# Parskatt/RoMa

Hardware: NVIDIA H100
Metric: image-pairs/sec match()+sample() 560->864 (higher is better)
Workload: dtype f32 (activations f32; GEMM operands as split-f16 pairs hi + 2^-11 lo on wgmma, f32 accumulate: fp32-class)

## Files before the change

include/romab200.h:

```cpp
#ifndef ROMAB200_H
#define ROMAB200_H

#include <stdint.h>

#ifdef __cplusplus
extern "C" {
#endif

#define ROMAB200_ABI_VERSION 4

enum rb_dtype { RB_F32 = 0, RB_F16 = 1, RB_BF16 = 2, RB_F16S = 3, RB_F64 = 4 };
enum rb_act { RB_ACT_NONE = 0, RB_ACT_RELU = 1, RB_ACT_GELU = 2 };
enum rb_rowmap { RB_ROWMAP_NONE = 0, RB_ROWMAP_PAD_KEEP = 1, RB_ROWMAP_PAD_TO_COMPACT = 2, RB_ROWMAP_SEGMENT = 3 };
enum rb_epi { RB_EPI_LINEAR = 0, RB_EPI_COSKERNEL = 1 };
enum rb_backend { RB_BACKEND_AUTO = 0, RB_BACKEND_SIMT = 1, RB_BACKEND_TCGEN05 = 2 };

int romab200_abi_version(void);
const char* romab200_last_error(void);
unsigned long long romab200_launch_count(void);
int romab200_device_ok(void);

typedef struct {
    const void* A; const void* B; void* C;
    int32_t M, N, K;
// ... 39 lines not shown

typedef struct {
    const void* src; void* dst; int64_t rows; int32_t cols; int64_t lds, ldd; int32_t dtype_src, dtype_dst;
    const float* row_scale; int32_t row_scale_reciprocal;
} rb_copy2d_args;
int romab200_copy2d(const rb_copy2d_args* args, void* stream);

typedef struct {
    const void* src; void* dst; const int32_t* src_index; const int32_t* dst_index;
    int32_t count; int64_t row_bytes, ld_src, ld_dst; int32_t src_rows, dst_rows;
} rb_gather_rows_args;
int romab200_gather_rows(const rb_gather_rows_args* args, void* stream);

typedef struct {
    const float* x; void* dst; int64_t rows; int32_t cols; int64_t ldx, ldd; const float* row_norm;
    int32_t layout_b;
} rb_split_args;
int romab200_split_f16x3(const rb_split_args* args, void* stream);

typedef struct {
    const float* x; void* hi; void* lo; int64_t rows; int32_t cols; int64_t ldx, ldd; const float* row_norm;
} rb_split_pair_args;
int romab200_split_f16s(const rb_split_pair_args* args, void* stream);

typedef struct {
    const float* image; void* out; const float* weight ; const float* bias ;
    int32_t batch, height, width, cout; int32_t dtype_out;
    void* out_lo;
} rb_conv_first_args;
int romab200_conv3x3_first(const rb_conv_first_args* args, void* stream);
typedef struct { const void* in; void* out; int32_t batch, height, width, channels, dtype;
                 const void* in_lo; void* out_lo;  } rb_maxpool_args;
int romab200_maxpool2x2_padded(const rb_maxpool_args* args, void* stream);

typedef struct { const float* image; void* out; int32_t batch, height, width, patch; int64_t ldo; int32_t dtype_out; } rb_im2col_args;
int romab200_im2col_patch(const rb_im2col_args* args, void* stream);
typedef struct { const float* patch; const float* cls; const float* pos; float* tokens; int32_t batch, npatch, dim; } rb_tokens_args;
int romab200_assemble_tokens(const rb_tokens_args* args, void* stream);

typedef struct {
    float* W; int32_t n, nrhs, batch; int64_t ldw, stride;
    void* workspace; int64_t workspace_bytes;
    int32_t algo;
} rb_gp_solve_args;
int romab200_gp_solve(const rb_gp_solve_args* args, void* stream);
typedef struct { const void* logits; float* state; int64_t rows; int64_t ldl; int32_t res; int32_t dtype; } rb_cls_args;
int romab200_cls_to_flow_refine(const rb_cls_args* args, void* stream);

typedef struct {
    const void* feat; int64_t ldf; int32_t n_img, y_shift;
    const float* state; void* d; int64_t ldd;
    int32_t D, h, w, cf, emb, radius; int32_t dtype;
    const float* emb_weight ; const float* emb_bias; float disp_scale;
    const float* grid_x; const float* grid_y;
    const float* win_x; const float* win_y;
    void* tile_done; int32_t tile_done_len;
    const float* corr_table; int64_t ld_corr_table;
} rb_refiner_prologue_args;
int romab200_refiner_prologue(const rb_refiner_prologue_args* args, void* stream);

typedef struct {
    const void* f0; const void* f1; int64_t ldf0, ldf1; int64_t f0_img_stride, f1_img_stride;
    const float* flow; int64_t ldflow; void* out; int64_t ldo;
    int32_t batch, h, w, c, radius; float scale; int32_t dtype_f, dtype_out;
    int32_t n_img, y_shift;
    const float* win_x; const float* win_y;
// ... 543 lines not shown
```

roma_b200/cabi.py:

```python
from __future__ import annotations

import ctypes
import os
import re
from typing import Dict

import torch

HERE = os.path.dirname(os.path.abspath(__file__))
HEADER = os.path.join(os.path.dirname(HERE), "include", "romab200.h")
LIB_PATH = os.path.join(HERE, "lib", "libromab200.so")

RB_F32, RB_F16, RB_BF16, RB_F16S, RB_F64 = 0, 1, 2, 3, 4
ACT_NONE, ACT_RELU, ACT_GELU = 0, 1, 2
ROWMAP_NONE, ROWMAP_PAD_KEEP, ROWMAP_PAD_TO_COMPACT, ROWMAP_SEGMENT = 0, 1, 2, 3
EPI_LINEAR, EPI_COSKERNEL = 0, 1
BACKEND_AUTO, BACKEND_SIMT, BACKEND_TCGEN05 = 0, 1, 2
SAMPLE_IDENTITY, SAMPLE_THRESHOLD, SAMPLE_BALANCE = 0, 1, 2

DTYPE_CODE = {torch.float32: RB_F32, torch.float16: RB_F16, torch.bfloat16: RB_BF16}

_CTYPES = {
    "int32_t": ctypes.c_int32, "int64_t": ctypes.c_int64, "uint64_t": ctypes.c_uint64, "float": ctypes.c_float, "double": ctypes.c_double,
}
# ... 66 lines not shown
                           "(there is no CPU or PyTorch fallback for the CUDA path)")
    lib = ctypes.CDLL(path)
    lib.romab200_last_error.restype = ctypes.c_char_p
    lib.romab200_abi_version.restype = ctypes.c_int
    lib.romab200_device_ok.restype = ctypes.c_int
    lib.romab200_launch_count.restype = ctypes.c_ulonglong
    for fn in FUNCTIONS:
        getattr(lib, fn)
    _lib = lib
    return lib


def _stream():
    return ctypes.c_void_p(torch.cuda.current_stream().cuda_stream)


launch_count = 0

_CODE_DTYPE = {RB_F32: torch.float32, RB_F16: torch.float16, RB_BF16: torch.bfloat16, RB_F16S: torch.float16, RB_F64: torch.float64}
_F32 = torch.float32
_F64 = torch.float64
_FIELD_DTYPES = {
    "rb_gemm_args": {"A": "dtype_ab", "B": "dtype_ab", "A_lo": torch.float16, "B_lo": torch.float16, "C": "dtype_c", "C_lo": torch.float16,
                     "R": "dtype_r", "bias": _F32, "col_scale": _F32, "norm_a": _F32, "norm_b": _F32},
    "rb_layernorm_args": {"x": "dtype_x", "y": "dtype_y", "y_lo": torch.float16, "gamma": _F32, "beta": _F32},
    "rb_softmax_args": {"s": "dtype", "out_hi": torch.float16, "out_lo": torch.float16},
    "rb_flash_attn_args": {"qkv": "dtype", "out": "dtype", "qkv_lo": torch.float16, "out_lo": torch.float16},
    "rb_rownorm_args": {"x": "dtype", "out": _F32},
    "rb_copy2d_args": {"src": "dtype_src", "dst": "dtype_dst", "row_scale": _F32},
    "rb_gather_rows_args": {"src_index": torch.int32, "dst_index": torch.int32},
    "rb_split_pair_args": {"x": _F32, "hi": torch.float16, "lo": torch.float16, "row_norm": _F32},
    "rb_conv_first_args": {"image": _F32, "out": "dtype_out", "out_lo": torch.float16, "weight": _F32, "bias": _F32},
    "rb_maxpool_args": {"in": "dtype", "out": "dtype", "in_lo": torch.float16, "out_lo": torch.float16},
    "rb_im2col_args": {"image": _F32, "out": "dtype_out"},
    "rb_tokens_args": {"patch": _F32, "cls": _F32, "pos": _F32, "tokens": _F32},
    "rb_gp_solve_args": {"W": _F32},
    "rb_cls_args": {"logits": "dtype", "state": _F32},
    "rb_refiner_prologue_args": {"feat": "dtype", "state": _F32, "d": "dtype", "emb_weight": _F32, "emb_bias": _F32, "grid_x": _F32, "grid_y": _F32,
                                 "win_x": _F32, "win_y": _F32, "tile_done": torch.uint8, "corr_table": _F32},
    "rb_local_corr_args": {"f0": "dtype_f", "f1": "dtype_f", "flow": _F32, "out": "dtype_out", "win_x": _F32, "win_y": _F32},
    "rb_local_corr_warp_args": {"f0": _F32, "f1": _F32, "warp": _F32, "out": _F32},
    "rb_dwconv_args": {"in": "dtype", "weight": _F32, "bias": _F32, "out_lo": torch.float16},
    "rb_refiner_block_small_args": {"in": "dtype", "out": "dtype", "dw_weight": _F32, "dw_bias": _F32, "pw_weight_host": _F32, "pw_bias_host": _F32},
    "rb_refiner_block_c144_args": {"in": "dtype", "out": "dtype", "dw_weight": _F32, "dw_bias": _F32, "pw_weight": "dtype", "pw_bias": _F32},
    "rb_refiner_block_c144_split_args": {"in": _F32, "out": _F32, "dw_weight": _F32, "dw_bias": _F32, "pw_weight": torch.float16,
                                         "pw_weight_lo": torch.float16, "pw_bias": _F32},
    "rb_refiner_tail_args": {"d": "dtype", "weight": _F32, "bias": _F32, "state": _F32, "delta_out": _F32},
    "rb_resize_args": {"in": _F32, "out": _F32},
    "rb_match_epilogue_args": {"state": _F32, "coarse_state": _F32, "warp": _F32, "cert": _F32, "grid_x": _F32, "grid_y": _F32},
    "rb_kde_args": {"x": _F32, "density": _F32, "workspace": _F32},
    "rb_preprocess_args": {"in": torch.uint8, "tmp": torch.uint8, "out_u8": torch.uint8, "out": _F32, "bounds_x": torch.int32, "kk_x": torch.int32,
                           "bounds_y": torch.int32, "kk_y": torch.int32},
    "rb_sample_args": {"values": _F32, "out_idx": torch.int32, "out_weights": _F32, "keys": _F32, "scratch": torch.int32, "seed_dev": torch.int64},
    "rb_sample_gather_args": {"matches": _F32, "certainty": _F32, "idx": torch.int32, "out_matches": _F32, "out_certainty": _F32},
    "rb_tiny_conv_args": {"in": _F32, "out": _F32, "weight": _F32, "bias": _F32, "col_scale": _F32, "R": _F32},
    "rb_tiny_gray_args": {"in": _F32, "out": _F32},
    "rb_tiny_avgpool_args": {"in": _F32, "out": _F32},
    "rb_tiny_add3_args": {"a": _F32, "b": _F32, "c": _F32, "out": _F32},
    "rb_tiny_pos_embed_args": {"f0": _F32, "f1": _F32, "state": _F32, "grid_x": _F32, "grid_y": _F32, "grid_lr_x": _F32, "grid_lr_y": _F32},
    "rb_tiny_warp_concat_args": {"f0": _F32, "f1": _F32, "state": _F32, "out": _F32},
    "rb_tiny_epilogue_args": {"state": _F32, "warp": _F32, "cert": _F32, "grid_x": _F32, "grid_y": _F32},
    "rb_keypoints_sample_args": {"x": _F32, "warp": _F32, "cert": _F32, "x_to_B": _F32, "cert_out": _F32},
    "rb_keypoints_mnn_args": {"x_A_to_B": _F32, "cert_A": _F32, "x_B": _F32, "workspace": _F32, "offsets": torch.int64, "inds_A": torch.int64,
                              "inds_B": torch.int64},
    "rb_jpeg_args": {"stream": torch.uint8, "desc": torch.int64, "tables": torch.int32, "comp": torch.uint8, "chunks": torch.int32,
                     "istart": torch.int32, "exits": torch.int64, "counts": torch.int32, "coef": torch.int16, "state": torch.int32,
# ... 45 lines not shown
                        "x2": _F64, "prob": _F32},
    "rb_dense_geometric_dist_args": {"depth0": "depth_dtype", "depth1": "depth_dtype", "T": _F64, "K0": _F64, "K1": _F64, "dense_matches": _F32,
                                     "gd": _F64, "prob": _F32, "partial_sum": _F64, "partial_cnt": torch.int32, "pair_sum": _F64,
                                     "pair_cnt": torch.int64, "pck": _F32, "epe": _F64},
    "rb_dense_tri_args": {"pairs": torch.int64, "warp": _F32, "certainty": _F32, "image_sizes": torch.int32, "cameras": _F64,
                          "registered": torch.uint8, "images": torch.int32, "depth": _F32, "score": _F32, "source": torch.int64,
                          "elem_depth": _F32, "partial": torch.int32, "pair_counts": torch.int64},
    "rb_dense_fuse_args": {"image_sizes": torch.int32, "cameras": _F64, "registered": torch.uint8, "nbr_offsets": torch.int64,
                           "nbrs": torch.int32, "depth": _F32, "score": _F32, "colors": torch.uint8, "color_offsets": torch.int64,
                           "color_sizes": torch.int32, "tile_scan": torch.int64, "points": _F64, "rgb": torch.uint8, "image": torch.int32,
                           "pixel": torch.int64, "num_views": torch.int32, "point_score": _F32},
}
_STRIDED_FIELDS = {"rb_keypoints_sample_args": {"warp", "cert"}, "rb_dense_geometric_dist_args": {"dense_matches"}}
_HOST_FIELDS = {"rb_refiner_block_small_args": {"pw_weight_host", "pw_bias_host"}}


def _gemm_min_elems(kw):
    b0, b1 = kw.get("batch0", 1) or 1, kw.get("batch1", 1) or 1
    M, N, K, nt = kw["M"], kw["N"], kw["K"], kw.get("ntaps", 1) or 1
    offa = (b0 - 1) * kw.get("sa0", 0) + (b1 - 1) * kw.get("sa1", 0)
    offb = (b0 - 1) * kw.get("sb0", 0) + (b1 - 1) * kw.get("sb1", 0)
    offc = (b0 - 1) * kw.get("sc0", 0) + (b1 - 1) * kw.get("sc1", 0)
    a = offa + ((kw.get("a_rows") or M) - 1) * kw["lda"] + K // nt
    b = offb + ((K - 1) * kw["ldb"] + N if kw.get("trans_b", 0) else (N - 1) * kw["ldb"] + K)
    rows_out = M
    if kw.get("rowmap", 0) == ROWMAP_PAD_TO_COMPACT:
        rows_out = M // (kw["pad_h"] * kw["pad_w"]) * (kw["pad_h"] - 2) * (kw["pad_w"] - 2)
    elif kw.get("rowmap", 0) == ROWMAP_SEGMENT:
        rows_out = (M - 1) // kw["seg_in"] * kw["seg_out"] + (M - 1) % kw["seg_in"] + kw.get("seg_off", 0) + 1
    c = offc + (rows_out - 1) * kw["ldc"] + N
    return {"A": a, "A_lo": a, "B": b, "B_lo": b, "C": c, "C_lo": c}


def _copy2d_min_elems(kw):
    return {"src": (kw["rows"] - 1) * kw["lds"] + kw["cols"], "dst": (kw["rows"] - 1) * kw["ldd"] + kw["cols"]}


def _gather_rows_min_elems(kw):
    out = {}
    for k, rows, ld in (("src", "src_rows", "ld_src"), ("dst", "dst_rows", "ld_dst")):
        if isinstance(kw.get(k), torch.Tensor):
            out[k] = -(-((kw[rows] - 1) * kw[ld] + kw["row_bytes"]) // kw[k].element_size())
    return out


def _sample_min_elems(kw):
    b, n, k, rep = max(kw.get("batch", 1), 1), kw["n"], kw["k"], max(kw.get("repeats", 0), 1)
    return {"values": ((b - 1) // rep) * (kw.get("stride") or n) + n, "keys": b * n, "scratch": b * 2056, "out_idx": b * k, "out_weights": b * k,
            "seed_dev": (b - 1) * kw.get("seed_stride", 0) + 1}


def _sample_gather_min_elems(kw):
    items, k, rows = kw["items"], kw["k"], ((kw["items"] - 1) // max(kw.get("repeats", 0), 1) + 1) * kw["n"]
    return {"matches": 4 * rows, "certainty": rows, "idx": items * k, "out_matches": 4 * items * k, "out_certainty": items * k}


def _match_graph_keypoints_min_elems(kw):
    sides, img = kw["num_pairs"] * kw["n"], kw["num_images"] + 1
    return {"pairs": 2 * kw["num_pairs"], "matches": 4 * sides, "certainty": sides, "image_sizes": 2 * kw["num_images"], "cell_start": img,
            "tile_start": img, "grid_bits": kw["grid_cells"], "grid_g": kw["grid_cells"], "tile_scan": kw["grid_tiles"] + 1, "kp_offsets": img,
            "keypoints": 2 * kw["kp_capacity"], "kp_scores": kw["kp_capacity"], "sid": 2 * sides}


def _match_graph_pairs_min_elems(kw):
    sides, cap = kw["num_pairs"] * kw["n"], kw.get("match_capacity", 0)
    return {"sid": 2 * sides, "certainty": sides, "scratch": kw.get("scratch_bytes", 0), "match_offsets": kw["num_pairs"] + 1,
# ... 64 lines not shown
        total = kw["x"].numel() // 2
        out.update(images=kw["num_list"], out_offsets=kw["num_list"] + 1, X=3 * total)
    return out


def _undistort_min_elems(kw):
    return {"kp_offsets": kw["num_images"] + 1, "keypoints": 2 * kw["num_rows"], "intrinsics": 4 * kw["num_images"], "out": 2 * kw["num_rows"],
            "clamped": 1}


def _twoview_min_elems(kw):
    B, total = kw["batch"], kw["mask"].numel()
    return {"offsets": B + 1, "x0": 2 * total, "x1": 2 * total, "xn": 4 * total, "K": 18 * B, "R": 9 * B, "t": 3 * B, "ok": B,
            "angle": total, "num_good": B, "median_angle": B, "forward": B}


def _dense_tri_min_elems(kw):
    P, N, C, n = kw["num_pairs"], kw["num_images"], kw["chunk"], kw["H"] * kw["W"]
    return {"pairs": 2 * P, "warp": 8 * C * n, "certainty": 2 * C * n, "image_sizes": 2 * N, "cameras": N * RB_DENSE_CAM, "registered": N,
            "images": kw["num_list"], "depth": N * n, "score": N * n, "source": N * n, "elem_depth": 2 * C * n,
            "partial": 2 * C * RB_DENSE_MAX_CTAS * RB_DENSE_REASONS, "pair_counts": P * RB_DENSE_REASONS}


def _dense_fuse_min_elems(kw):
    N, n, M = kw["num_images"], kw["H"] * kw["W"], kw.get("num_points", 0)
    out = {"image_sizes": 2 * N, "cameras": N * RB_DENSE_CAM, "registered": N, "nbr_offsets": N + 1, "depth": N * n, "score": N * n,
           "color_offsets": N + 1, "color_sizes": 2 * N, "tile_scan": N * (-(-n // RB_DENSE_TILE)) + 1, "points": 3 * M, "rgb": 3 * M,
           "image": M, "pixel": M, "num_views": M, "point_score": M}
    if kw.get("colors") is not None:
        out["colors"] = kw["color_bytes"]
    return out


_MIN_ELEMS = {"rb_gemm_args": _gemm_min_elems, "rb_copy2d_args": _copy2d_min_elems, "rb_gather_rows_args": _gather_rows_min_elems,
              "rb_sample_args": _sample_min_elems, "rb_sample_gather_args": _sample_gather_min_elems,
              "rb_match_graph_keypoints_args": _match_graph_keypoints_min_elems, "rb_match_graph_pairs_args": _match_graph_pairs_min_elems,
              "rb_tracks_args": _tracks_min_elems, "rb_verify_args": _verify_min_elems, "rb_tri_args": _tri_min_elems,
              "rb_ba_args": _ba_min_elems, "rb_ba_groups_args": _ba_groups_min_elems, "rb_abspose_args": _abspose_min_elems,
              "rb_register_args": _register_min_elems,
              "rb_twoview_args": _twoview_min_elems, "rb_undistort_args": _undistort_min_elems,
              "rb_dense_tri_args": _dense_tri_min_elems, "rb_dense_fuse_args": _dense_fuse_min_elems}


def _validate(fn_name, struct_name, kw):
    table = _FIELD_DTYPES.get(struct_name, {})
    cur = torch.cuda.current_device() if torch.cuda.is_available() else None
    mins = _MIN_ELEMS[struct_name](kw) if struct_name in _MIN_ELEMS else {}
    strided = _STRIDED_FIELDS.get(struct_name, ())
    host = _HOST_FIELDS.get(struct_name, ())
    for k, v in kw.items():
        if not isinstance(v, torch.Tensor):
            if v is not None and k in _PTR_FIELDS[struct_name]:
                raise TypeError(f"{fn_name}: pointer field `{k}` takes a tensor or None, not {type(v).__name__} "
                                "(pass an operand that starts inside a buffer as a view, packing.at)")
            continue
        if k in host:
            if v.device.type != "cpu":
                raise RuntimeError(f"{fn_name}: argument `{k}` is read on the host, it must be a CPU tensor (got one on {v.device})")
        elif not v.is_cuda or (cur is not None and v.device.index != cur):
            raise RuntimeError(f"{fn_name}: argument `{k}` lives on {v.device}, expected the current CUDA device cuda:{cur}")
        if k not in strided and not v.is_contiguous():
            raise RuntimeError(f"{fn_name}: argument `{k}` is not contiguous (shape {tuple(v.shape)}, strides {v.stride()})")
        want = table.get(k)
        if isinstance(want, str):
            want = _CODE_DTYPE.get(kw.get(want))
        if want is not None and v.dtype != want:
            raise RuntimeError(f"{fn_name}: argument `{k}` has dtype {v.dtype}, the call describes it as {want}")
# ... 40 lines not shown
```

roma_b200/csrc/gemm_tc.cu:

```cuda
#include "tma.cuh"
#include "wgmma.cuh"

namespace rb {

struct TcParams {
    int M, N, K;
    int batch1;
    int ntaps, k_per_tap; int tap_rows[9];
    int tiles_m, tiles_n, total_tiles;
    int band_m;
    int n_zero_to;
    int64_t sc0, sc1, sr0, sr1, sna0, snb0;
    Epilogue epi;
};

constexpr int TC_BM = 128, TC_BK = 64;
constexpr int TC_THREADS = 384;
constexpr int TC_CW = 32, TC_SP = 40;
constexpr int TC_STAGING = 2 * 64 * TC_SP * 4;

template <int BN, bool SPLIT> struct TcCfg {
    static constexpr int NOPS = SPLIT ? 2 : 1;
    static constexpr int A_BYTES = TC_BM * TC_BK * 2;
    static constexpr int B_BYTES = BN * TC_BK * 2;
// ... 85 lines not shown
            v[k] = expf((v[k] * s - 1.0f) * e.inv_t);
            if (m == n + k) v[k] += e.diag_add;
        }
    } else {
#pragma unroll
        for (int k = 0; k < 8; ++k) v[k] = __fmul_rn(e.alpha, v[k]);
        if (e.bias) {
#pragma unroll
            for (int k = 0; k < 8; ++k) v[k] = __fadd_rn(v[k], cb[k]);
        }
        if (e.act == RB_ACT_RELU) {
#pragma unroll
            for (int k = 0; k < 8; ++k) v[k] = fmaxf(v[k], 0.0f);
        } else if (e.act == RB_ACT_GELU) {
#pragma unroll
            for (int k = 0; k < 8; ++k) v[k] = gelu_erf(v[k]);
        }
        if (e.col_scale) {
#pragma unroll
            for (int k = 0; k < 8; ++k) v[k] = __fmul_rn(v[k], cs[k]);
        }
        if (e.R) {
            float r[8];
            load8(e.R, orow * e.ldr + n, e.dtype_r, nv, r);
#pragma unroll
            for (int k = 0; k < 8; ++k) v[k] = __fadd_rn(v[k], r[k]);
        }
    }
    if (nv < 8) {
#pragma unroll
        for (int k = 0; k < 8; ++k) if (k >= nv) v[k] = 0.f;
    }
    store8(e, orow * e.ldc + n, cnt, v);
}

__device__ __forceinline__ void tile_coords(const TcParams& p, int w, int& z, int& mt, int& nt) {
    const int per_z = p.tiles_m * p.tiles_n;
    z = w / per_z;
    const int r = w - z * per_z;
    const int m_lo = r / (p.band_m * p.tiles_n) * p.band_m;
    const int rows = min(p.band_m, p.tiles_m - m_lo);
    const int rb = r - m_lo * p.tiles_n;
    nt = rb / rows;
    mt = m_lo + (rb - nt * rows);
}

template <int BN, bool SPLIT, bool BF16, int TB>
__global__ void __launch_bounds__(TC_THREADS, 1)
gemm_tc_kernel(const __grid_constant__ CUtensorMap map_a, const __grid_constant__ CUtensorMap map_b,
               const __grid_constant__ CUtensorMap map_a_lo, const __grid_constant__ CUtensorMap map_b_lo, const TcParams p) {
    using Cfg = TcCfg<BN, SPLIT>;
    constexpr int STAGES = Cfg::STAGES;
    constexpr int A_BYTES = Cfg::A_BYTES, B_BYTES = Cfg::B_BYTES;
    constexpr int OFF_A_LO = A_BYTES, OFF_B = Cfg::NOPS * A_BYTES, OFF_B_LO = Cfg::NOPS * A_BYTES + B_BYTES;
    extern __shared__ uint8_t smem_raw[];
    uint8_t* smem = smem_raw + ((1024u - ((uint32_t)__cvta_generic_to_shared(smem_raw) & 1023u)) & 1023u);
    float* staging = reinterpret_cast<float*>(smem + STAGES * Cfg::STAGE_BYTES);
    uint64_t* full_bar = reinterpret_cast<uint64_t*>(smem + STAGES * Cfg::STAGE_BYTES + TC_STAGING);
    uint64_t* empty_bar = full_bar + STAGES;

    const int warp = threadIdx.x >> 5, lane = threadIdx.x & 31;
    const int kblocks = (p.K + TC_BK - 1) / TC_BK;

    if (threadIdx.x == 0) {
        for (int s = 0; s < STAGES; ++s) { mbar_init(&full_bar[s], 1); mbar_init(&empty_bar[s], 2); }
        asm volatile("fence.mbarrier_init.release.cluster;" ::: "memory");
// ... 53 lines not shown
            wgmma_fence();
#pragma unroll
            for (int k = 0; k < TC_BK / 16; ++k) {
                const uint32_t koff_a = wg * (64 * 128) + k * 32;
                const uint32_t koff_b = TB ? k * 2048 : k * 32;
                const uint32_t lbo_b = TB ? 64 * 128 : 16;
                const uint64_t a_hi = gmma_desc(st + koff_a, 16, 1024);
                const uint64_t b_hi = gmma_desc(st + OFF_B + koff_b, lbo_b, 1024);
                const int accum = (kb | k) != 0;
                Wgmma<BN, BF16>::template ss<TB>(acc, a_hi, b_hi, accum);
                if constexpr (SPLIT) {
                    const uint64_t a_lo = gmma_desc(st + OFF_A_LO + koff_a, 16, 1024);
                    const uint64_t b_lo = gmma_desc(st + OFF_B_LO + koff_b, lbo_b, 1024);
                    Wgmma<BN, BF16>::template ss<TB>(acc2, a_hi, b_lo, accum);
                    Wgmma<BN, BF16>::template ss<TB>(acc2, a_lo, b_hi, 1);
                }
            }
            wgmma_commit();
            wgmma_wait<1>();
            if (prev >= 0 && t == 0) mbar_arrive(&empty_bar[prev]);
            prev = s;
        }
        wgmma_wait<0>();
        wgmma_fence_regs(acc);
        if constexpr (SPLIT) wgmma_fence_regs(acc2);
        if (t == 0) mbar_arrive(&empty_bar[prev]);

        Epilogue e = p.epi;
        e.C = (char*)e.C + (z0 * p.sc0 + z1 * p.sc1) * dtype_size(e.dtype_c);
        if (e.C_lo) e.C_lo = (char*)e.C_lo + (z0 * p.sc0 + z1 * p.sc1) * 2;
        if (e.R) e.R = (const char*)e.R + (z0 * p.sr0 + z1 * p.sr1) * dtype_size(e.dtype_r);
        if (e.norm_a) e.norm_a += z0 * p.sna0;
        if (e.norm_b) e.norm_b += z0 * p.snb0;
        float* stg = staging + wg * (64 * TC_SP);
        const int fr = (t >> 5) * 16 + ((t & 31) >> 2), fc = 2 * (t & 3);
        const int g = t & 3, rr = t >> 2;
        int mrow[2]; int64_t orow[2]; float na[2] = {0.f, 0.f};
#pragma unroll
        for (int h = 0; h < 2; ++h) {
            mrow[h] = m0 + wg * 64 + rr + 32 * h;
            orow[h] = mrow[h] < e.M ? e.map_row(mrow[h]) : -1;
            if (orow[h] >= 0 && e.epi == RB_EPI_COSKERNEL) na[h] = e.norm_a[mrow[h]];
        }
        constexpr int NCH = (BN + TC_CW - 1) / TC_CW;
#pragma unroll 1
        for (int ch = 0; ch < NCH; ++ch) {
            if (n0 + ch * TC_CW >= p.n_zero_to) break;
            bar_named(1 + wg, 128);
#pragma unroll
            for (int c = 0; c < NCH; ++c) {
                if (c != ch) continue;
#pragma unroll
                for (int jj = 0; jj < TC_CW / 8; ++jj) {
                    const int j = c * (TC_CW / 8) + jj;
                    if (j >= BN / 8) break;
#pragma unroll
                    for (int h = 0; h < 2; ++h) {
                        float v0 = acc[4 * j + 2 * h], v1 = acc[4 * j + 2 * h + 1];
                        if constexpr (SPLIT) {
                            v0 = fmaf(acc2[4 * j + 2 * h], 1.0f / RB_SPLIT_SCALE, v0);
                            v1 = fmaf(acc2[4 * j + 2 * h + 1], 1.0f / RB_SPLIT_SCALE, v1);
                        }
                        *reinterpret_cast<float2*>(stg + (fr + 8 * h) * TC_SP + 8 * jj + fc) = make_float2(v0, v1);
                    }
                }
            }
            bar_named(1 + wg, 128);
            const int n = n0 + ch * TC_CW + 8 * g;
            if (ch * TC_CW + 8 * g >= BN || n >= p.n_zero_to) continue;
            const int cnt = min(8, p.n_zero_to - n);
            float cb[8], cs[8];
            const float* colb = e.epi == RB_EPI_COSKERNEL ? e.norm_b : e.bias;
#pragma unroll
            for (int k = 0; k < 8; ++k) {
                const bool in = n + k < e.N;
                cb[k] = colb && in ? colb[n + k] : 0.f;
                cs[k] = e.col_scale && in ? e.col_scale[n + k] : 0.f;
            }
#pragma unroll
            for (int h = 0; h < 2; ++h) {
                if (orow[h] < 0) continue;
                const float* src = stg + (rr + 32 * h) * TC_SP + 8 * g;
                const int q = (rr & 1) * 4;
                const float4 a = *reinterpret_cast<const float4*>(src + q), b = *reinterpret_cast<const float4*>(src + (4 - q));
                float v[8];
                if (q == 0) { v[0] = a.x; v[1] = a.y; v[2] = a.z; v[3] = a.w; v[4] = b.x; v[5] = b.y; v[6] = b.z; v[7] = b.w; }
                else        { v[0] = b.x; v[1] = b.y; v[2] = b.z; v[3] = b.w; v[4] = a.x; v[5] = a.y; v[6] = a.z; v[7] = a.w; }
                epilogue8(e, mrow[h], n, orow[h], cnt, cb, cs, na[h], v);
            }
        }
    }
}

static int make_map(CUtensorMap* map, const void* base, int dtype, uint64_t inner, uint64_t rows, uint64_t pitch_elems, uint64_t b1,
                    uint64_t s1_elems, uint64_t b0, uint64_t s0_elems, uint32_t box_inner, uint32_t box_rows) {
    RB_REQUIRE(((uintptr_t)base) % 16 == 0 && (pitch_elems * 2) % 16 == 0, "gemm_tc: operand base/pitch must be 16-byte aligned (pitch %llu elems)", (unsigned long long)pitch_elems);
    RB_REQUIRE((b1 <= 1 || (s1_elems * 2) % 16 == 0) && (b0 <= 1 || (s0_elems * 2) % 16 == 0), "gemm_tc: batch strides must be 16-byte aligned");
    cuuint64_t dims[4] = {inner, rows, b1 > 0 ? b1 : 1, b0 > 0 ? b0 : 1};
    cuuint64_t strides[3] = {pitch_elems * 2, (b1 > 1 ? s1_elems : pitch_elems * rows) * 2, (b0 > 1 ? s0_elems : pitch_elems * rows) * 2};
    cuuint32_t box[4] = {box_inner, box_rows, 1, 1};
    return encode_tiled(map, "gemm_tc", tma_dtype(dtype), 4, base, dims, strides, box,
                        CU_TENSOR_MAP_SWIZZLE_128B);
}

struct TcMaps { CUtensorMap a, b, a_lo, b_lo; };

template <int BN, bool SPLIT, bool BF16, int TB>
static int launch_tc(const TcMaps& maps, TcParams& p, int zdim, int max_ctas, cudaStream_t st) {
    using Cfg = TcCfg<BN, SPLIT>;
    auto kernel = gemm_tc_kernel<BN, SPLIT, BF16, TB>;
    if (ensure_smem<gemm_tc_kernel<BN, SPLIT, BF16, TB>>(Cfg::SMEM, "gemm_tc")) return 1;
    p.tiles_m = (p.M + TC_BM - 1) / TC_BM;
    p.tiles_n = (p.N + BN - 1) / BN;
    const long long total = (long long)p.tiles_m * p.tiles_n * zdim;
    RB_REQUIRE(total < (1ll << 31), "gemm_tc: too many tiles");
    p.total_tiles = (int)total;
    int resident = sm_count();
    if (max_ctas > 0 && max_ctas < resident) resident = max_ctas;
    const int grid = p.total_tiles < resident ? p.total_tiles : resident;
    const int64_t a_bytes = (int64_t)p.M * (p.ntaps > 1 ? p.k_per_tap : p.K) * Cfg::NOPS * 2;
    const int64_t b_bytes = (int64_t)p.N * p.K * Cfg::NOPS * 2;
    const bool bands = p.tiles_n > 1 && 2 * a_bytes > l2_bytes() && 2 * b_bytes <= l2_bytes();
// ... 52 lines not shown
        else if (a->N <= 144) BN = 144;
        else if (a->N <= 192) BN = 192;
        else {
            const int w192 = (a->N + 191) / 192 * 192 - a->N, w256 = (a->N + 255) / 256 * 256 - a->N;
            BN = (w192 + a->N / 20 < w256) ? 192 : 256;
        }
        if (((int64_t)((a->M + 127) / 128) * ((a->N + BN - 1) / BN) * zdim) < sm_count() * 2 / 3) BN = 128;
    }
    TcMaps maps;
    const uint64_t a_inner = p.ntaps > 1 ? p.k_per_tap : a->K;
    if (make_map(&maps.a, a->A, a->dtype_ab, a_inner, a_rows, a->lda, p.batch1, a->sa1, batch0, a->sa0, TC_BK, TC_BM)) return 1;
    if (split && make_map(&maps.a_lo, a->A_lo, a->dtype_ab, a_inner, a_rows, a->lda, p.batch1, a->sa1, batch0, a->sa0, TC_BK, TC_BM)) return 1;
    if (!a->trans_b) {
        if (make_map(&maps.b, a->B, a->dtype_ab, a->K, a->N, a->ldb, p.batch1, a->sb1, batch0, a->sb0, TC_BK, BN)) return 1;
        if (split && make_map(&maps.b_lo, a->B_lo, a->dtype_ab, a->K, a->N, a->ldb, p.batch1, a->sb1, batch0, a->sb0, TC_BK, BN)) return 1;
    } else {
        if (make_map(&maps.b, a->B, a->dtype_ab, a->N, a->K, a->ldb, p.batch1, a->sb1, batch0, a->sb0, 64, TC_BK)) return 1;
        if (split && make_map(&maps.b_lo, a->B_lo, a->dtype_ab, a->N, a->K, a->ldb, p.batch1, a->sb1, batch0, a->sb0, 64, TC_BK)) return 1;
    }
    if (!split) { maps.a_lo = maps.a; maps.b_lo = maps.b; }
    {
        const int es_c = dtype_size(a->dtype_c);
        const bool align_ok = ((uintptr_t)a->C) % 16 == 0 && (a->ldc * es_c) % 16 == 0 && (p.batch1 <= 1 || (a->sc1 * es_c) % 16 == 0) &&
                              (batch0 <= 1 || (a->sc0 * es_c) % 16 == 0) && (a->dtype_c != RB_F16S || ((uintptr_t)a->C_lo) % 16 == 0);
        const bool rowmap_ok = a->rowmap == RB_ROWMAP_NONE || a->rowmap == RB_ROWMAP_PAD_KEEP;
        const int gran = 16 / es_c;
        p.n_zero_to = align_ok && rowmap_ok && !a->R ? (a->N + gran - 1) / gran * gran : a->N;
    }
    if (split) return dispatch_tc<true, false>(BN, a->trans_b, maps, p, zdim, a->max_ctas, stream);
    return bf16 ? dispatch_tc<false, true>(BN, a->trans_b, maps, p, zdim, a->max_ctas, stream)
                : dispatch_tc<false, false>(BN, a->trans_b, maps, p, zdim, a->max_ctas, stream);
}

}
```

roma_b200/engine.py:

```python
from __future__ import annotations

import math
import os
from contextlib import contextmanager
from typing import Optional

import torch
import torch.nn.functional as F

from . import arch, cabi, sampling
from .cabi import call
from .cache import BufferArena
from .packing import PackedWeights, Split, at, pad8

PRECISIONS = {"fp32": torch.float32, "fp32_simt": torch.float32, "fp16": torch.float16, "bf16": torch.bfloat16}
F16S = cabi.RB_F16S


class Engine(BufferArena):
    def __init__(self, matcher_sd, dino_sd, device, precision: str = "fp32"):
        if precision not in PRECISIONS:
            raise ValueError(f"precision must be one of {list(PRECISIONS)}")
        super().__init__(device)
        if self.device.type != "cuda":
# ... 80 lines not shown
        if self._lane == "side" and self.side_ctas:
            args["max_ctas"] = self.side_ctas
        args.update(kw)
        if (self.split and dtype_ab is None) or isinstance(A, Split):
            if not isinstance(A, Split):
                assert args["batch0"] * args["batch1"] == 1 and lda % 8 == 0, "batched fp32 operands are split by the caller"
                A = self.split_pair(A, args.get("a_rows") or M, K // args["ntaps"], lda)
            if not isinstance(B, Split):
                assert args["batch0"] * args["batch1"] == 1 and ldb % 8 == 0
                tb = args.get("trans_b", 0)
                B = self.split_pair(B, K if tb else N, N if tb else K, ldb, name=f"splitb.{self._lane}.{(K if tb else N) * ldb}")
            dtype_ab = F16S
            args.update(A=A.hi, A_lo=A.lo, B=B.hi, B_lo=B.lo)
            if isinstance(C, Split):
                args.update(C=C.hi, C_lo=C.lo)
                dtype_c = F16S
            else:
                args.update(C=C)
        else:
            args.update(A=A, B=B, C=C)
        args["dtype_ab"] = self.dt if dtype_ab is None else dtype_ab
        args["dtype_c"] = self.dt if dtype_c is None else dtype_c
        if self.gemm_profile is None:
            call("romab200_gemm", "rb_gemm_args", **args)
            return
        start, end = torch.cuda.Event(enable_timing=True), torch.cuda.Event(enable_timing=True)
        start.record()
        call("romab200_gemm", "rb_gemm_args", **args)
        end.record()
        flops = 2.0 * M * N * K * args["batch0"] * args["batch1"]
        backend = {cabi.RB_F32: "simt", F16S: "tcgen05-split"}.get(args["dtype_ab"], "tcgen05")
        self.gemm_profile.append((backend, flops, start, end, (M, N, K, args["batch0"] * args["batch1"]), args.get("epi", cabi.EPI_LINEAR)))

    def layernorm(self, x, y, gb, rows, cols, eps, dtype_y=None):
        if isinstance(y, Split):
            call("romab200_layernorm", "rb_layernorm_args", x=x, y=y.hi, y_lo=y.lo, gamma=gb[0], beta=gb[1], rows=rows, cols=cols,
                 ldx=cols, ldy=cols, dtype_x=cabi.RB_F32, dtype_y=F16S, eps=eps)
            return
        call("romab200_layernorm", "rb_layernorm_args", x=x, y=y, gamma=gb[0], beta=gb[1], rows=rows, cols=cols,
             ldx=cols, ldy=cols, dtype_x=cabi.RB_F32, dtype_y=self.dt if dtype_y is None else dtype_y, eps=eps)

    def copy2d(self, src, dst, rows, cols, lds, ldd, ds, dd):
        call("romab200_copy2d", "rb_copy2d_args", src=src, dst=dst, rows=rows, cols=cols, lds=lds, ldd=ldd,
             dtype_src=ds, dtype_dst=dd)

    def vgg(self, image: torch.Tensor, tag: str):
        E, _, H, W = image.shape
        taps = {}
        layers = self.w.vgg
        h, w = H, W
        mk = (lambda name, shape: self.sbuf(name, shape, zero=True)) if self.split else (lambda name, shape: self.buf(name, shape, zero=True))
        cur = mk(f"vgg{tag}.s1.in", (E, h + 2, w + 2, 64))
        if self.split:
            call("romab200_conv3x3_first", "rb_conv_first_args", image=image, out=cur.hi, out_lo=cur.lo, weight=layers[0]["w"], bias=layers[0]["b"],
                 batch=E, height=h, width=w, cout=64, dtype_out=F16S)
        else:
            call("romab200_conv3x3_first", "rb_conv_first_args", image=image, out=cur, weight=layers[0]["w"], bias=layers[0]["b"],
                 batch=E, height=h, width=w, cout=64, dtype_out=self.dt)
        li, scale = 1, 1
        for nconv in (1, 2, 4, 4):
            for j in range(nconv):
                L = layers[li]
                li += 1
                nxt = mk(f"vgg{tag}.s{scale}.p{j % 2}", (E, h + 2, w + 2, L["cout"]))
                rows = E * (h + 2) * (w + 2)
                taps_rows = [(ky - 1) * (w + 2) + (kx - 1) for ky in range(3) for kx in range(3)]
                self.gemm(cur, L["w"], nxt, rows, L["cout"], 9 * L["cin"], L["cin"], 9 * L["cin"], L["cout"],
                          ntaps=9, tap_rows=taps_rows, a_rows=rows, bias=L["b"], act=cabi.ACT_RELU,
                          rowmap=cabi.ROWMAP_PAD_KEEP, pad_h=h + 2, pad_w=w + 2)
                cur = nxt
            taps[scale] = (cur, h, w)
            if self.debug is not None:
                self.debug[f"{tag}.vgg{scale}"] = (cur.join() if self.split else cur.float())[:, 1:h + 1, 1:w + 1].clone()
            if scale == 8:
                break
            c = layers[li - 1]["cout"]
            pooled = mk(f"vgg{tag}.s{scale * 2}.in", (E, h // 2 + 2, w // 2 + 2, c))
            if self.split:
                call("romab200_maxpool2x2_padded", "rb_maxpool_args", **{"in": cur.hi}, in_lo=cur.lo, out=pooled.hi, out_lo=pooled.lo,
                     batch=E, height=h, width=w, channels=c, dtype=F16S)
            else:
                call("romab200_maxpool2x2_padded", "rb_maxpool_args", **{"in": cur}, out=pooled, batch=E, height=h, width=w,
                     channels=c, dtype=self.dt)
            cur, h, w, scale = pooled, h // 2, w // 2, scale * 2
        return taps

    def attention(self, qkv, out, Bn, N, heads, dim, tag):
        d = dim // heads
        if self.dtype != torch.float32 and self.use_flash_attn:
            with self.stage(f"  attn.{tag}"):
                call("romab200_flash_attn", "rb_flash_attn_args", qkv=qkv, out=out, ld_qkv=3 * dim, ld_out=dim, batch=Bn, n_tokens=N,
                     heads=heads, head_dim=d, dtype=self.dt)
            return
        npad = pad8(N)
        ld = 3 * dim
        if self.split and d == 64 and self.use_flash_attn:
            with self.stage(f"  attn.{tag}"):
                call("romab200_flash_attn", "rb_flash_attn_args", qkv=qkv.hi, qkv_lo=qkv.lo, out=out.hi, out_lo=out.lo, ld_qkv=ld, ld_out=dim,
                     batch=Bn, n_tokens=N, heads=heads, head_dim=d, dtype=F16S)
            return
        if self.split:
            S = self.buf(f"attn.scores.{tag}", (Bn, heads, N, npad), dtype=torch.float32)
# ... 433 lines not shown
```

Baseline: 17.63.

## Add halo-tiled implicit-GEMM conv3x3 kernel for split-f16 VGG layers

Adds a dedicated wgmma conv3x3 kernel for VGG layers with cin 64 or 128. Each CTA loads one spatial 8x16 halo tile (hi and lo planes) into shared memory once via 4D TMA and reuses it across all nine taps and all output-channel tiles. Weights stream through an mbarrier ring driven by a producer warp. The goal is to cut redundant global re-reads of the A operand that the generic tap-row GEMM does per tap. The shared epilogue is factored into a helper. Risks are shared-memory pressure limiting stage depth, and wasted work on partial tiles at image edges.

New measurement: 17.75 (median of 6 runs). Within noise of the previous version (+0.7%).

```diff
diff --git a/include/romab200.h b/include/romab200.h
--- a/include/romab200.h
+++ b/include/romab200.h
@@ -95,6 +95,16 @@
 typedef struct { const void* in; void* out; int32_t batch, height, width, channels, dtype;
                  const void* in_lo; void* out_lo;  } rb_maxpool_args;
 int romab200_maxpool2x2_padded(const rb_maxpool_args* args, void* stream);
+typedef struct {
+    const void* in; const void* in_lo;
+    const void* weight; const void* weight_lo;
+    const float* bias;
+    void* out; void* out_lo;
+    int32_t batch, height, width, cin, cout;
+    int32_t act;
+    int32_t max_ctas;
+} rb_conv3x3_split_args;
+int romab200_conv3x3_split(const rb_conv3x3_split_args* args, void* stream);
 
 typedef struct { const float* image; void* out; int32_t batch, height, width, patch; int64_t ldo; int32_t dtype_out; } rb_im2col_args;
 int romab200_im2col_patch(const rb_im2col_args* args, void* stream);
diff --git a/roma_b200/cabi.py b/roma_b200/cabi.py
--- a/roma_b200/cabi.py
+++ b/roma_b200/cabi.py
@@ -122,6 +122,8 @@
     "rb_split_pair_args": {"x": _F32, "hi": torch.float16, "lo": torch.float16, "row_norm": _F32},
     "rb_conv_first_args": {"image": _F32, "out": "dtype_out", "out_lo": torch.float16, "weight": _F32, "bias": _F32},
     "rb_maxpool_args": {"in": "dtype", "out": "dtype", "in_lo": torch.float16, "out_lo": torch.float16},
+    "rb_conv3x3_split_args": {"in": torch.float16, "in_lo": torch.float16, "weight": torch.float16, "weight_lo": torch.float16, "bias": _F32,
+                              "out": torch.float16, "out_lo": torch.float16},
     "rb_im2col_args": {"image": _F32, "out": "dtype_out"},
     "rb_tokens_args": {"patch": _F32, "cls": _F32, "pos": _F32, "tokens": _F32},
     "rb_gp_solve_args": {"W": _F32},
@@ -233,6 +235,12 @@
     return {"A": a, "A_lo": a, "B": b, "B_lo": b, "C": c, "C_lo": c}
 
 
+def _conv3x3_split_min_elems(kw):
+    pix = kw["batch"] * (kw["height"] + 2) * (kw["width"] + 2)
+    a, w, c = pix * kw["cin"], 9 * kw["cin"] * kw["cout"], pix * kw["cout"]
+    return {"in": a, "in_lo": a, "weight": w, "weight_lo": w, "bias": kw["cout"], "out": c, "out_lo": c}
+
+
 def _copy2d_min_elems(kw):
     return {"src": (kw["rows"] - 1) * kw["lds"] + kw["cols"], "dst": (kw["rows"] - 1) * kw["ldd"] + kw["cols"]}
 
@@ -363,7 +371,7 @@
     return out
 
 
-_MIN_ELEMS = {"rb_gemm_args": _gemm_min_elems, "rb_copy2d_args": _copy2d_min_elems, "rb_gather_rows_args": _gather_rows_min_elems,
+_MIN_ELEMS = {"rb_gemm_args": _gemm_min_elems, "rb_conv3x3_split_args": _conv3x3_split_min_elems, "rb_copy2d_args": _copy2d_min_elems, "rb_gather_rows_args": _gather_rows_min_elems,
               "rb_sample_args": _sample_min_elems, "rb_sample_gather_args": _sample_gather_min_elems,
               "rb_match_graph_keypoints_args": _match_graph_keypoints_min_elems, "rb_match_graph_pairs_args": _match_graph_pairs_min_elems,
               "rb_tracks_args": _tracks_min_elems, "rb_verify_args": _verify_min_elems, "rb_tri_args": _tri_min_elems,
diff --git a/roma_b200/csrc/gemm_tc.cu b/roma_b200/csrc/gemm_tc.cu
--- a/roma_b200/csrc/gemm_tc.cu
+++ b/roma_b200/csrc/gemm_tc.cu
@@ -141,6 +141,61 @@
         for (int k = 0; k < 8; ++k) if (k >= nv) v[k] = 0.f;
     }
     store8(e, orow * e.ldc + n, cnt, v);
+}
+
+template <int BN, bool SPLIT>
+__device__ __forceinline__ void tile_epilogue(const Epilogue& e, const float (&acc)[BN / 2], const float (&acc2)[SPLIT ? BN / 2 : 1], float* stg,
+                                              int wg, int t, int n0, int n_zero_to, const int (&mrow)[2], const int64_t (&orow)[2],
+                                              const float (&na)[2]) {
+    const int fr = (t >> 5) * 16 + ((t & 31) >> 2), fc = 2 * (t & 3);
+    const int g = t & 3, rr = t >> 2;
+    constexpr int NCH = (BN + TC_CW - 1) / TC_CW;
+#pragma unroll 1
+    for (int ch = 0; ch < NCH; ++ch) {
+        if (n0 + ch * TC_CW >= n_zero_to) break;
+        bar_named(1 + wg, 128);
+#pragma unroll
+        for (int c = 0; c < NCH; ++c) {
+            if (c != ch) continue;
+#pragma unroll
+            for (int jj = 0; jj < TC_CW / 8; ++jj) {
+                const int j = c * (TC_CW / 8) + jj;
+                if (j >= BN / 8) break;
+#pragma unroll
+                for (int h = 0; h < 2; ++h) {
+                    float v0 = acc[4 * j + 2 * h], v1 = acc[4 * j + 2 * h + 1];
+                    if constexpr (SPLIT) {
+                        v0 = fmaf(acc2[4 * j + 2 * h], 1.0f / RB_SPLIT_SCALE, v0);
+                        v1 = fmaf(acc2[4 * j + 2 * h + 1], 1.0f / RB_SPLIT_SCALE, v1);
+                    }
+                    *reinterpret_cast<float2*>(stg + (fr + 8 * h) * TC_SP + 8 * jj + fc) = make_float2(v0, v1);
+                }
+            }
+        }
+        bar_named(1 + wg, 128);
+        const int n = n0 + ch * TC_CW + 8 * g;
+        if (ch * TC_CW + 8 * g >= BN || n >= n_zero_to) continue;
+        const int cnt = min(8, n_zero_to - n);
+        float cb[8], cs[8];
+        const float* colb = e.epi == RB_EPI_COSKERNEL ? e.norm_b : e.bias;
+#pragma unroll
+        for (int k = 0; k < 8; ++k) {
+            const bool in = n + k < e.N;
+            cb[k] = colb && in ? colb[n + k] : 0.f;
+            cs[k] = e.col_scale && in ? e.col_scale[n + k] : 0.f;
+        }
+#pragma unroll
+        for (int h = 0; h < 2; ++h) {
+            if (orow[h] < 0) continue;
+            const float* src = stg + (rr + 32 * h) * TC_SP + 8 * g;
+            const int q = (rr & 1) * 4;
+            const float4 a = *reinterpret_cast<const float4*>(src + q), b = *reinterpret_cast<const float4*>(src + (4 - q));
+            float v[8];
+            if (q == 0) { v[0] = a.x; v[1] = a.y; v[2] = a.z; v[3] = a.w; v[4] = b.x; v[5] = b.y; v[6] = b.z; v[7] = b.w; }
+            else        { v[0] = b.x; v[1] = b.y; v[2] = b.z; v[3] = b.w; v[4] = a.x; v[5] = a.y; v[6] = a.z; v[7] = a.w; }
+            epilogue8(e, mrow[h], n, orow[h], cnt, cb, cs, na[h], v);
+        }
+    }
 }
 
 __device__ __forceinline__ void tile_coords(const TcParams& p, int w, int& z, int& mt, int& nt) {
@@ -260,9 +315,7 @@
         if (e.R) e.R = (const char*)e.R + (z0 * p.sr0 + z1 * p.sr1) * dtype_size(e.dtype_r);
         if (e.norm_a) e.norm_a += z0 * p.sna0;
         if (e.norm_b) e.norm_b += z0 * p.snb0;
-        float* stg = staging + wg * (64 * TC_SP);
-        const int fr = (t >> 5) * 16 + ((t & 31) >> 2), fc = 2 * (t & 3);
-        const int g = t & 3, rr = t >> 2;
+        const int rr = t >> 2;
         int mrow[2]; int64_t orow[2]; float na[2] = {0.f, 0.f};
 #pragma unroll
         for (int h = 0; h < 2; ++h) {
@@ -270,52 +323,147 @@
             orow[h] = mrow[h] < e.M ? e.map_row(mrow[h]) : -1;
             if (orow[h] >= 0 && e.epi == RB_EPI_COSKERNEL) na[h] = e.norm_a[mrow[h]];
         }
-        constexpr int NCH = (BN + TC_CW - 1) / TC_CW;
+        tile_epilogue<BN, SPLIT>(e, acc, acc2, staging + wg * (64 * TC_SP), wg, t, n0, p.n_zero_to, mrow, orow, na);
+    }
+}
+
+constexpr int CV_BW = 8, CV_BH = 16;
+constexpr int CV_HW = CV_BW + 2, CV_HH = CV_BH + 2;
+constexpr int CV_HALO_PIX = CV_HW * CV_HH;
+
+struct ConvParams {
+    int E, H, W, cin, cout;
+    int tiles_x, tiles_y, tiles_n, total_tiles;
+    Epilogue epi;
+};
+
+template <int BN, int CIN> struct ConvCfg {
+    static constexpr int CG_BYTES = (CV_HALO_PIX * 16 + 127) / 128 * 128;
+    static constexpr int HALO_BYTES = CIN / 8 * CG_BYTES;
+    static constexpr int HALO_TX = CIN / 8 * CV_HALO_PIX * 16;
+    static constexpr int B_BYTES = BN * TC_BK * 2;
+    static constexpr int STAGE_BYTES = 2 * B_BYTES;
+    static constexpr int NHALO = (232448 - 4 * HALO_BYTES - TC_STAGING - 1024 - 256) / STAGE_BYTES >= 4 ? 2 : 1;
+    static constexpr int RING_MAX = 232448 - NHALO * 2 * HALO_BYTES - TC_STAGING - 1024  - 256 ;
+    static constexpr int STAGES = RING_MAX / STAGE_BYTES > 8 ? 8 : RING_MAX / STAGE_BYTES;
+    static constexpr int SMEM = STAGES * STAGE_BYTES + NHALO * 2 * HALO_BYTES + TC_STAGING + 1024 + 256;
+    static_assert(STAGES >= 3 && SMEM <= 232448, "shared memory budget");
+};
+
+template <int BN, int CIN>
+__global__ void __launch_bounds__(TC_THREADS, 1)
+conv3x3_tc_kernel(const __grid_constant__ CUtensorMap map_in, const __grid_constant__ CUtensorMap map_in_lo,
+                  const __grid_constant__ CUtensorMap map_w, const __grid_constant__ CUtensorMap map_w_lo, const ConvParams p) {
+    using Cfg = ConvCfg<BN, CIN>;
+    constexpr int STAGES = Cfg::STAGES, B_BYTES = Cfg::B_BYTES, HALO_BYTES = Cfg::HALO_BYTES;
+    constexpr int KB_PER_TAP = CIN / TC_BK, KBLOCKS = 9 * KB_PER_TAP;
+    constexpr int CG_BYTES = Cfg::CG_BYTES, NHALO = Cfg::NHALO;
+    extern __shared__ uint8_t smem_raw[];
+    uint8_t* smem = smem_raw + ((1024u - ((uint32_t)__cvta_generic_to_shared(smem_raw) & 1023u)) & 1023u);
+    uint8_t* halo = smem + STAGES * Cfg::STAGE_BYTES;
+    float* staging = reinterpret_cast<float*>(halo + NHALO * 2 * HALO_BYTES);
+    uint64_t* full_bar = reinterpret_cast<uint64_t*>(halo + NHALO * 2 * HALO_BYTES + TC_STAGING);
+    uint64_t* empty_bar = full_bar + STAGES;
+    uint64_t* halo_full = empty_bar + STAGES;
+    uint64_t* halo_empty = halo_full + NHALO;
+
+    const int warp = threadIdx.x >> 5, lane = threadIdx.x & 31;
+    const int per_img = p.tiles_x * p.tiles_y;
+    if (threadIdx.x == 0) {
+        for (int s = 0; s < STAGES; ++s) { mbar_init(&full_bar[s], 1); mbar_init(&empty_bar[s], 2); }
+        for (int b = 0; b < NHALO; ++b) { mbar_init(&halo_full[b], 1); mbar_init(&halo_empty[b], 2); }
+        asm volatile("fence.mbarrier_init.release.cluster;" ::: "memory");
+    }
+    __syncthreads();
+    rb::pdl_wait();
+
+    if (warp >= 8) {
+        asm volatile("setmaxnreg.dec.sync.aligned.u32 40;");
+        if (warp == 8 && lane == 0) {
+            uint32_t it = 0, tc = 0;
+            for (int tile = blockIdx.x; tile < p.total_tiles; tile += gridDim.x, ++tc) {
+                const int img = tile / per_img, r = tile - img * per_img;
+                const int by = r / p.tiles_x, bx = r - by * p.tiles_x;
+                const int hb = tc % NHALO;
+                uint8_t* hal = halo + hb * 2 * HALO_BYTES;
+                mbar_wait(&halo_empty[hb], ((tc / NHALO) & 1) ^ 1);
+                mbar_expect_tx(&halo_full[hb], 2 * Cfg::HALO_TX);
 #pragma unroll 1
-        for (int ch = 0; ch < NCH; ++ch) {
-            if (n0 + ch * TC_CW >= p.n_zero_to) break;
-            bar_named(1 + wg, 128);
-#pragma unroll
-            for (int c = 0; c < NCH; ++c) {
-                if (c != ch) continue;
-#pragma unroll
-                for (int jj = 0; jj < TC_CW / 8; ++jj) {
-                    const int j = c * (TC_CW / 8) + jj;
-                    if (j >= BN / 8) break;
-#pragma unroll
-                    for (int h = 0; h < 2; ++h) {
-                        float v0 = acc[4 * j + 2 * h], v1 = acc[4 * j + 2 * h + 1];
-                        if constexpr (SPLIT) {
-                            v0 = fmaf(acc2[4 * j + 2 * h], 1.0f / RB_SPLIT_SCALE, v0);
-                            v1 = fmaf(acc2[4 * j + 2 * h + 1], 1.0f / RB_SPLIT_SCALE, v1);
-                        }
-                        *reinterpret_cast<float2*>(stg + (fr + 8 * h) * TC_SP + 8 * jj + fc) = make_float2(v0, v1);
+                for (int c = 0; c < CIN / 8; ++c) {
+                    tma_load_4d(hal + c * CG_BYTES, &map_in, &halo_full[hb], 8 * c, bx * CV_BW, by * CV_BH, img);
+                    tma_load_4d(hal + HALO_BYTES + c * CG_BYTES, &map_in_lo, &halo_full[hb], 8 * c, bx * CV_BW, by * CV_BH, img);
+                }
+                for (int nt = 0; nt < p.tiles_n; ++nt) {
+                    for (int kb = 0; kb < KBLOCKS; ++kb, ++it) {
+                        const int s = it % STAGES;
+                        mbar_wait(&empty_bar[s], ((it / STAGES) & 1) ^ 1);
+                        mbar_expect_tx(&full_bar[s], Cfg::STAGE_BYTES);
+                        uint8_t* st = smem + s * Cfg::STAGE_BYTES;
+                        tma_load_4d(st, &map_w, &full_bar[s], kb * TC_BK, nt * BN, 0, 0);
+                        tma_load_4d(st + B_BYTES, &map_w_lo, &full_bar[s], kb * TC_BK, nt * BN, 0, 0);
                     }
                 }
             }
-            bar_named(1 + wg, 128);
-            const int n = n0 + ch * TC_CW + 8 * g;
-            if (ch * TC_CW + 8 * g >= BN || n >= p.n_zero_to) continue;
-            const int cnt = min(8, p.n_zero_to - n);
-            float cb[8], cs[8];
-            const float* colb = e.epi == RB_EPI_COSKERNEL ? e.norm_b : e.bias;
-#pragma unroll
-            for (int k = 0; k < 8; ++k) {
-                const bool in = n + k < e.N;
-                cb[k] = colb && in ? colb[n + k] : 0.f;
-                cs[k] = e.col_scale && in ? e.col_scale[n + k] : 0.f;
+        }
+        return;
+    }
+
+    asm volatile("setmaxnreg.inc.sync.aligned.u32 232;");
+    const int wg = warp >> 2, t = threadIdx.x & 127;
+    const uint32_t halo_u32 = smem_u32(halo);
+    float acc[BN / 2];
+    float acc2[BN / 2];
+    uint32_t it = 0, tc = 0;
+    for (int tile = blockIdx.x; tile < p.total_tiles; tile += gridDim.x, ++tc) {
+        const int img = tile / per_img, r = tile - img * per_img;
+        const int by = r / p.tiles_x, bx = r - by * p.tiles_x;
+        const int rr = t >> 2;
+        int mrow[2]; int64_t orow[2]; const float na[2] = {0.f, 0.f};
+#pragma unroll
+        for (int h = 0; h < 2; ++h) {
+            const int lr = rr + 32 * h;
+            const int y = by * CV_BH + wg * 8 + lr / CV_BW, x = bx * CV_BW + lr % CV_BW;
+            orow[h] = y < p.H && x < p.W ? ((int64_t)img * (p.H + 2) + y + 1) * (p.W + 2) + x + 1 : -1;
+            mrow[h] = (int)orow[h];
+        }
+        const int hb = tc % NHALO;
+        const uint32_t hal_u32 = halo_u32 + hb * 2 * HALO_BYTES;
+        mbar_wait(&halo_full[hb], (tc / NHALO) & 1);
+        for (int nt = 0; nt < p.tiles_n; ++nt) {
+            int prev = -1;
+            for (int kb = 0; kb < KBLOCKS; ++kb, ++it) {
+                const int s = it % STAGES;
+                mbar_wait(&full_bar[s], (it / STAGES) & 1);
+                const uint32_t st = smem_u32(smem + s * Cfg::STAGE_BYTES);
+                const int tap = kb / KB_PER_TAP, cb = kb - tap * KB_PER_TAP;
+                const int ky = tap / 3, kx = tap - 3 * ky;
+                const uint32_t a0 = hal_u32 + ((wg * 8 + ky) * CV_HW + kx) * 16 + cb * 8 * CG_BYTES;
+                wgmma_fence();
+#pragma unroll
+                for (int k = 0; k < TC_BK / 16; ++k) {
+                    const uint32_t koff_a = 2 * k * CG_BYTES;
+                    const uint64_t a_hi = gmma_desc(a0 + koff_a, CG_BYTES, CV_HW * 16, 0);
+                    const uint64_t b_hi = gmma_desc(st + k * 32, 16, 1024);
+                    const int accum = (kb | k) != 0;
+                    Wgmma<BN, false>::template ss<0>(acc, a_hi, b_hi, accum);
+                    const uint64_t a_lo = gmma_desc(a0 + HALO_BYTES + koff_a, CG_BYTES, CV_HW * 16, 0);
+                    const uint64_t b_lo = gmma_desc(st + B_BYTES + k * 32, 16, 1024);
+                    Wgmma<BN, false>::template ss<0>(acc2, a_hi, b_lo, accum);
+                    Wgmma<BN, false>::template ss<0>(acc2, a_lo, b_hi, 1);
+                }
+                wgmma_commit();
+                wgmma_wait<1>();
+                if (prev >= 0 && t == 0) mbar_arrive(&empty_bar[prev]);
+                prev = s;
             }
-#pragma unroll
-            for (int h = 0; h < 2; ++h) {
-                if (orow[h] < 0) continue;
-                const float* src = stg + (rr + 32 * h) * TC_SP + 8 * g;
-                const int q = (rr & 1) * 4;
-                const float4 a = *reinterpret_cast<const float4*>(src + q), b = *reinterpret_cast<const float4*>(src + (4 - q));
-                float v[8];
-                if (q == 0) { v[0] = a.x; v[1] = a.y; v[2] = a.z; v[3] = a.w; v[4] = b.x; v[5] = b.y; v[6] = b.z; v[7] = b.w; }
-                else        { v[0] = b.x; v[1] = b.y; v[2] = b.z; v[3] = b.w; v[4] = a.x; v[5] = a.y; v[6] = a.z; v[7] = a.w; }
-                epilogue8(e, mrow[h], n, orow[h], cnt, cb, cs, na[h], v);
+            wgmma_wait<0>();
+            wgmma_fence_regs(acc);
+            wgmma_fence_regs(acc2);
+            if (t == 0) {
+                mbar_arrive(&empty_bar[prev]);
+                if (nt == p.tiles_n - 1) mbar_arrive(&halo_empty[hb]);
             }
+            tile_epilogue<BN, true>(p.epi, acc, acc2, staging + wg * (64 * TC_SP), wg, t, nt * BN, p.cout, mrow, orow, na);
         }
     }
 }
@@ -434,4 +582,61 @@
                 : dispatch_tc<false, false>(BN, a->trans_b, maps, p, zdim, a->max_ctas, stream);
 }
 
-}
+static int make_halo_map(CUtensorMap* map, const void* base, int E, int H, int W, int C) {
+    RB_REQUIRE(((uintptr_t)base) % 16 == 0, "conv3x3_split: input planes must be 16-byte aligned");
+    cuuint64_t dims[4] = {(cuuint64_t)C, (cuuint64_t)W + 2, (cuuint64_t)H + 2, (cuuint64_t)E};
+    cuuint64_t strides[3] = {(cuuint64_t)C * 2, (cuuint64_t)(W + 2) * C * 2, (cuuint64_t)(H + 2) * (W + 2) * C * 2};
+    cuuint32_t box[4] = {8, CV_HW, CV_HH, 1};
+    return encode_tiled(map, "conv3x3_split", CU_TENSOR_MAP_DATA_TYPE_FLOAT16, 4, base, dims, strides, box, CU_TENSOR_MAP_SWIZZLE_NONE);
+}
+
+template <int BN, int CIN>
+static int launch_conv(const TcMaps& maps, const ConvParams& p, int max_ctas, cudaStream_t st) {
+    using Cfg = ConvCfg<BN, CIN>;
+    auto kernel = conv3x3_tc_kernel<BN, CIN>;
+    if (ensure_smem<conv3x3_tc_kernel<BN, CIN>>(Cfg::SMEM, "conv3x3_split")) return 1;
+    int resident = sm_count();
+    if (max_ctas > 0 && max_ctas < resident) resident = max_ctas;
+    const int grid = p.total_tiles < resident ? p.total_tiles : resident;
+    cudaError_t err = rb::launch_pdl(kernel, dim3(grid), dim3(TC_THREADS), Cfg::SMEM, st, maps.a, maps.a_lo, maps.b, maps.b_lo, p);
+    if (err != cudaSuccess) { set_error("conv3x3_split: launch failed: %s", cudaGetErrorString(err)); return 1; }
+    return check_launch("conv3x3_split");
+}
+
+}
+
+extern "C" int romab200_conv3x3_split(const rb_conv3x3_split_args* a, void* stream) {
+    using namespace rb;
+    RB_REQUIRE(a && a->in && a->in_lo && a->weight && a->weight_lo && a->out && a->out_lo, "conv3x3_split: null operand");
+    RB_REQUIRE(a->cin == 64 || a->cin == 128, "conv3x3_split: cin must be 64 or 128 (got %d)", a->cin);
+    RB_REQUIRE(a->cout > 0 && a->cout % 64 == 0, "conv3x3_split: cout must be a positive multiple of 64 (got %d)", a->cout);
+    RB_REQUIRE(a->batch > 0 && a->height > 0 && a->width > 0, "conv3x3_split: empty map (%d x %d x %d)", a->batch, a->height, a->width);
+    RB_REQUIRE(a->act == RB_ACT_NONE || a->act == RB_ACT_RELU, "conv3x3_split: act must be none or relu (got %d)", a->act);
+    RB_REQUIRE((int64_t)a->batch * (a->height + 2) * (a->width + 2) < (1ll << 31), "conv3x3_split: map too large");
+    RB_REQUIRE(((uintptr_t)a->out) % 16 == 0 && ((uintptr_t)a->out_lo) % 16 == 0 && ((uintptr_t)a->weight) % 16 == 0 &&
+               ((uintptr_t)a->weight_lo) % 16 == 0, "conv3x3_split: operands must be 16-byte aligned");
+    ConvParams p;
+    p.E = a->batch; p.H = a->height; p.W = a->width; p.cin = a->cin; p.cout = a->cout;
+    p.tiles_x = (a->width + CV_BW - 1) / CV_BW;
+    p.tiles_y = (a->height + CV_BH - 1) / CV_BH;
+    const int BN = a->cout % 128 == 0 ? 128 : 64;
+    p.tiles_n = a->cout / BN;
+    p.total_tiles = p.E * p.tiles_x * p.tiles_y;
+    Epilogue& e = p.epi;
+    memset(&e, 0, sizeof(e));
+    e.C = a->out; e.C_lo = a->out_lo; e.ldc = a->cout; e.dtype_c = RB_F16S;
+    e.alpha = 1.0f; e.bias = a->bias; e.act = a->act; e.epi = RB_EPI_LINEAR;
+    e.rowmap = RB_ROWMAP_PAD_KEEP; e.pad_h = a->height + 2; e.pad_w = a->width + 2;
+    e.M = a->batch * (a->height + 2) * (a->width + 2); e.N = a->cout;
+    TcMaps maps;
+    if (make_halo_map(&maps.a, a->in, p.E, p.H, p.W, p.cin) || make_halo_map(&maps.a_lo, a->in_lo, p.E, p.H, p.W, p.cin)) return 1;
+    if (make_map(&maps.b, a->weight, RB_F16S, 9 * a->cin, a->cout, 9 * a->cin, 1, 0, 1, 0, TC_BK, BN)) return 1;
+    if (make_map(&maps.b_lo, a->weight_lo, RB_F16S, 9 * a->cin, a->cout, 9 * a->cin, 1, 0, 1, 0, TC_BK, BN)) return 1;
+    cudaStream_t st = (cudaStream_t)stream;
+    if (a->cin == 64) return BN == 64 ? launch_conv<64, 64>(maps, p, a->max_ctas, st) : launch_conv<128, 64>(maps, p, a->max_ctas, st);
+    return BN == 64 ? launch_conv<64, 128>(maps, p, a->max_ctas, st) : launch_conv<128, 128>(maps, p, a->max_ctas, st);
+}
+
+namespace rb {
+
+}
diff --git a/roma_b200/engine.py b/roma_b200/engine.py
--- a/roma_b200/engine.py
+++ b/roma_b200/engine.py
@@ -136,6 +136,21 @@
         backend = {cabi.RB_F32: "simt", F16S: "tcgen05-split"}.get(args["dtype_ab"], "tcgen05")
         self.gemm_profile.append((backend, flops, start, end, (M, N, K, args["batch0"] * args["batch1"]), args.get("epi", cabi.EPI_LINEAR)))
 
+    def conv3x3_split(self, x: Split, L, y: Split, E, h, w):
+        kw = dict(**{"in": x.hi}, in_lo=x.lo, weight=L["w"].hi, weight_lo=L["w"].lo, bias=L["b"], out=y.hi, out_lo=y.lo,
+                  batch=E, height=h, width=w, cin=L["cin"], cout=L["cout"], act=cabi.ACT_RELU)
+        if self._lane == "side" and self.side_ctas:
+            kw["max_ctas"] = self.side_ctas
+        if self.gemm_profile is None:
+            call("romab200_conv3x3_split", "rb_conv3x3_split_args", **kw)
+            return
+        start, end = torch.cuda.Event(enable_timing=True), torch.cuda.Event(enable_timing=True)
+        start.record()
+        call("romab200_conv3x3_split", "rb_conv3x3_split_args", **kw)
+        end.record()
+        M, N, K = E * (h + 2) * (w + 2), L["cout"], 9 * L["cin"]
+        self.gemm_profile.append(("tcgen05-split", 2.0 * M * N * K, start, end, (M, N, K, 1), cabi.EPI_LINEAR))
+
     def layernorm(self, x, y, gb, rows, cols, eps, dtype_y=None):
         if isinstance(y, Split):
             call("romab200_layernorm", "rb_layernorm_args", x=x, y=y.hi, y_lo=y.lo, gamma=gb[0], beta=gb[1], rows=rows, cols=cols,
@@ -168,10 +183,13 @@
                 li += 1
                 nxt = mk(f"vgg{tag}.s{scale}.p{j % 2}", (E, h + 2, w + 2, L["cout"]))
                 rows = E * (h + 2) * (w + 2)
-                taps_rows = [(ky - 1) * (w + 2) + (kx - 1) for ky in range(3) for kx in range(3)]
-                self.gemm(cur, L["w"], nxt, rows, L["cout"], 9 * L["cin"], L["cin"], 9 * L["cin"], L["cout"],
-                          ntaps=9, tap_rows=taps_rows, a_rows=rows, bias=L["b"], act=cabi.ACT_RELU,
-                          rowmap=cabi.ROWMAP_PAD_KEEP, pad_h=h + 2, pad_w=w + 2)
+                if self.split and L["cin"] in (64, 128):
+                    self.conv3x3_split(cur, L, nxt, E, h, w)
+                else:
+                    taps_rows = [(ky - 1) * (w + 2) + (kx - 1) for ky in range(3) for kx in range(3)]
+                    self.gemm(cur, L["w"], nxt, rows, L["cout"], 9 * L["cin"], L["cin"], 9 * L["cin"], L["cout"],
+                              ntaps=9, tap_rows=taps_rows, a_rows=rows, bias=L["b"], act=cabi.ACT_RELU,
+                              rowmap=cabi.ROWMAP_PAD_KEEP, pad_h=h + 2, pad_w=w + 2)
                 cur = nxt
             taps[scale] = (cur, h, w)
             if self.debug is not None:
```
